# szuwgh/whisper.rs

Measured on AMD Instinct MI355X. Metric: real-time factor + encoder ms, Whisper-base 30s audio, 1 GPU and 8-GPU batch, higher is better.
Workload: dtype f16; 1 GPU; whisper-base f16 (random-init ggml-v1 weights), 1 x 30 s synthetic clip(s) per GPU: mel + conv stem + encoder + cross-KV + 128 greedy tokens; beam=0, clips_per_gpu=1, global_clips=1, n_decode=128, parallelism=1 GPU

## Files before the change

### whisper.rs_amd/csrc/wmi_api.cpp

```cpp
#include <hip/hip_runtime.h>
#include <rccl/rccl.h>

#include <math.h>
#include <stdarg.h>
#include <stdio.h>
#include <stdlib.h>
#include <string.h>

#include <algorithm>
#include <map>
#include <memory>
#include <set>
#include <string>
#include <vector>

#include "../../include/whisper_mi355x.h"
#include "wmi_host.h"
#include "wmi_internal.h"

#pragma clang fp contract(off)

using namespace wmi;

namespace {
// ... 113 lines not shown
    size_t tt_tsum_cap = 0;
    float *tt_pcm = nullptr;
    size_t tt_pcm_cap = 0;
    char *tt_spans = nullptr;
    size_t tt_spans_cap = 0;
    struct TokTime { int64_t t0, t1; float vlen; };
    struct Segment { int64_t t0, t1; int first, count; std::string text; };
    struct SegList {
        std::vector<Segment> segments;
        std::vector<TsRec> tokens;
        std::vector<TokTime> times;
    };
    std::vector<SegList> results = std::vector<SegList>(1);
    std::vector<int32_t> ts_prompt;
    int n_lang = 0;
    int task = WMI_TASK_TRANSCRIBE;
    std::vector<int32_t> lang_set;
    std::vector<int32_t> lang_used;
    std::vector<float> lang_p;
    bool lang_default = true, lang_any_auto = false;
    int32_t *d_lang = nullptr;
    int32_t *d_lang_auto = nullptr, *d_lang_det = nullptr;
    float *d_lang_p = nullptr, *d_lang_probs = nullptr;
    uint32_t *derr = nullptr;
    size_t sync_bytes = 0;
    int s_stride = 0, n_chunks_max = 0;
    unsigned long long *damax = nullptr;
    DecState *dstate = nullptr;
    int32_t *dfeed = nullptr;
    int feed_cap = 0;
    int32_t *dtokens = nullptr;
    size_t tokens_cap = 0;
    std::vector<float *> pcm_dev;
    std::vector<size_t> pcm_cap;
    float **d_pcm_ptrs = nullptr;
    int64_t *d_nsamp = nullptr, *d_nlen = nullptr;
    uint32_t *d_melmax = nullptr;
    float *d_mel = nullptr;
    size_t mel_cap = 0;
    int64_t mel_stride = 0, max_len = 0;
    std::vector<int64_t> n_len_host, n_samp_host;
    std::map<int32_t, float *> au_taps;
    void *au_raw = nullptr;
    float *au_mono = nullptr;
    size_t au_raw_cap = 0, au_mono_cap = 0;
    long long au_chunk = AUDIO_CHUNK_MAX;
    std::vector<hipEvent_t> au_ev;
    float au_ms = 0.0f;
    int au_converted = 0;
    int n_clips = 0;
    int enc_T = 0;
    int enc_clips = 0;
    int layout_T = -1;
    int cur_ctx = 0;
    int staged_n_decode = 0;
    std::vector<std::vector<int32_t>> staged_beam;
    hipEvent_t ev[8] = {};
    wmi_timings timings{};
    struct Graph { hipGraph_t graph = nullptr; hipGraphExec_t exec = nullptr; };
    std::map<std::string, Graph> graphs;
    void clear_graphs() {
        for (auto &kv : graphs) {
            if (kv.second.exec) (void)hipGraphExecDestroy(kv.second.exec);
            if (kv.second.graph) (void)hipGraphDestroy(kv.second.graph);
        }
        graphs.clear();
    }
    bool use_graph = true;
    bool use_coop = true;
    Tune tune;
    bool checksums = false;
    float cks[5] = {0, 0, 0, 0, 0};
    bool use_persist = true;
    int persist_q5 = -1;
    bool persist_logits = false;
    float *d_lgall = nullptr;
    int lg_rows = 0;
    int dec_layers = 0;
    int enc_layers = 0;
    int fault_inject = 0;
    bool persist_vreg = true;
    bool use_xshare = true;
    int early_ops = 1;
    int split_rows = 8;
    hipStream_t stream2 = nullptr;
    hipEvent_t ev_fork = nullptr, ev_join = nullptr;
    uint64_t *d_xg2 = nullptr;
    DecState *dstate2 = nullptr;
    int n_fallbacks = 0;
    PersistLayer *d_players = nullptr;
    uint32_t *d_expfb = nullptr;
    float gelu_min = __builtin_huge_valf();
    int n_expfb = 0;
    uint64_t *d_xg = nullptr;
    size_t xg_bytes = 0;
    int32_t *d_curtok = nullptr;
    int persist_G[9] = {-1, -1, -1, -1, -1, -1, -1, -1, -1};
    int persist_nres[9] = {};
    unsigned long long *d_ptrace = nullptr;
    ncclComm_t comm = nullptr;
    int rank = 0, world = 1;
    int32_t *d_gather = nullptr;
    int32_t *d_dsend = nullptr;
    int32_t *d_dctl = nullptr;
    int32_t *d_dbar = nullptr, *d_dshape = nullptr;
    size_t gather_cap = 0;
};

static float gelu_min_of(const wmi_context *ctx) { return ctx->tune.gelu_calc ? ctx->gelu_min : __builtin_huge_valf(); }

namespace {

int set_err(wmi_context *ctx, int code, const char *fmt, ...) {
    char buf[1024];
    va_list ap;
    va_start(ap, fmt);
    vsnprintf(buf, sizeof(buf), fmt, ap);
    va_end(ap);
    if (ctx) ctx->last_error = buf;
    g_last_error = buf;
    return code;
}

#define HIPCHK(ctx, expr)                                                                        \
    do {                                                                                         \
        hipError_t _e = (expr);                                                                  \
        if (_e != hipSuccess)                                                                    \
            return set_err((ctx), WMI_E_HIP, "HIP error %s at %s:%d: %s", hipGetErrorName(_e),    \
                           __FILE__, __LINE__, #expr);                                           \
    } while (0)

#define RCCLCHK(ctx, expr)                                                                       \
    do {                                                                                         \
        ncclResult_t _r = (expr);                                                                \
        if (_r != ncclSuccess)                                                                   \
            return set_err((ctx), WMI_E_RCCL, "RCCL error %s at %s:%d", ncclGetErrorString(_r),    \
                           __FILE__, __LINE__);                                                  \
    } while (0)

int prompt_tokens(const wmi_context *ctx, int32_t *out) {
    int n = 0;
    out[n++] = ctx->sp.sot;
    if (ctx->sp.is_multilingual) {
        out[n++] = ctx->sp.sot + 1;
        out[n++] = ctx->task == WMI_TASK_TRANSLATE ? ctx->sp.translate : ctx->sp.transcribe;
    }
    out[n++] = ctx->sp.not_;
    return n;
}

const char *const kLangCodes[LANG_MAX] = {
    "en", "zh", "de", "es", "ru", "ko", "fr", "ja", "pt", "tr", "pl", "ca", "nl", "ar", "sv", "it", "id", "hi", "fi", "vi",
    "he", "uk", "el", "ms", "cs", "ro", "da", "hu", "ta", "no", "th", "ur", "hr", "bg", "lt", "la", "mi", "ml", "cy", "sk",
    "te", "fa", "lv", "bn", "sr", "az", "sl", "kn", "et", "mk", "br", "eu", "is", "hy", "ne", "mn", "bs", "kk", "sq", "sw",
    "gl", "mr", "pa", "si", "km", "sn", "yo", "so", "af", "oc", "ka", "be", "tg", "sd", "gu", "am", "yi", "lo", "uz", "fo",
    "ht", "ps", "tk", "nn", "mt", "sa", "lb", "my", "bo", "tl", "mg", "as", "tt", "haw", "ln", "ha", "ba", "jw", "su", "yue",
};

struct Arena {
    size_t off = 0;
    std::vector<std::pair<size_t, size_t>> dummy;
    size_t take(size_t bytes) {
        const size_t o = off;
        off = up(off + bytes, 256);
        return o;
    }
// ... 1069 lines not shown
                    if (pd) pw[kk] += (double)((long long)pd - (long long)prev) * 0.01;
                    prev = v;
                }
            tot += (double)(prev - s0) * 0.01;
            ++ns;
        }
        if (!ns) return WMI_OK;
        double l1 = 0, l2 = 0, l3 = 0;
        for (int st = 1; st < steps; ++st) {
            const unsigned long long e = at(st, L - 1, 10, w);
            l1 += (double)(at(st, L, 1, w) - e) * 0.01;
            l2 += (double)(at(st, L, 2, w) - e) * 0.01;
            l3 += (double)(at(st, L, 3, w) - e) * 0.01;
        }
        fprintf(stderr, "[wmi ptrace] wg %s: logits LN done %.2f, resident rows done %.2f, streamed rows done %.2f us\n",
                wname[w], l1 / ns, l2 / ns, l3 / ns);
        if (steps > 2) {
            const double dc = (double)(at(steps - 1, L, 4, w) - at(1, L, 4, w));
            const double dt = (double)(at(steps - 1, L, 0, w) - at(1, L, 0, w)) * 10e-9;
            fprintf(stderr, "[wmi ptrace] wg %s: shader clock %.3f GHz\n", wname[w], dc / dt * 1e-9);
        }
        fprintf(stderr, "[wmi ptrace] wg %s: step %.2f us; per phase (per layer) total / until input arrived:\n", wname[w], tot / ns);
        for (int k = 0; k < 12; ++k) {
            const double d = k < 11 ? (double)ns * L : (double)ns;
            fprintf(stderr, "[wmi ptrace]   %-9s %6.2f / %6.2f\n", nm[k], ph[k] / d, pw[k] / d);
        }
        for (int k = 11; k < 32; ++k) {
            if (k == 16) k = 27;
            double s = 0;
            int c = 0;
            for (int st = 1; st < steps; ++st)
                for (int l = 0; l < L; ++l) {
                    const unsigned long long v = at(st, l, k, w);
                    unsigned long long pd = 0;
                    for (int j = 16; j < 27; ++j) {
                        const unsigned long long p = at(st, l, j, w);
                        if (p && p <= v && p > pd) pd = p;
                    }
                    if (v && pd) { s += (double)(v - pd) * 0.01; ++c; }
                }
            if (c) fprintf(stderr, "[wmi ptrace]   sub %d: %6.2f us after poll\n", k, s / c);
        }
    }
    return WMI_OK;
}

int persist_grid_for(wmi_context *ctx, int B) {
    if (!ctx->use_persist || B < 1 || B > 8) return 0;
    if (ctx->persist_G[B] < 0)
        ctx->persist_G[B] = persist_grid(ctx->device, ctx->hp.n_text_state, B, ctx->hp.n_audio_ctx, ctx->hp.n_vocab,
                                         &ctx->persist_nres[B]);
    return ctx->persist_G[B];
}

PersistArgs persist_args(wmi_context *ctx, const DecRun &run, int G) {
    const wmi_hparams &hp = ctx->hp;
    const int n = hp.n_text_state, H = hp.n_text_head, T = ctx->enc_T;
    const int b0 = run.b0, B = run.B, out_stride = run.out_stride;
    const bool beam = run.kind == RUN_BEAM;
    PersistArgs a{};
    a.layers = ctx->d_players; a.te = ctx->te; a.pe = ctx->d_pe; a.dln_w = ctx->dln_w; a.dln_b = ctx->dln_b;
    a.gelu_tab = ctx->gelu_tab; a.exp_tab = ctx->exp_tab; a.n_exp = ctx->n_exp; a.exp_fb = ctx->d_expfb;
    a.gelu_min = gelu_min_of(ctx);
    a.kcache = ctx->kcache; a.vcache = ctx->vcache; a.ck = ctx->ck; a.cv = ctx->cv;
    a.L = ctx->dec_layers; a.n = n; a.V = hp.n_vocab; a.B = B; a.T = T; a.tctx = hp.n_text_ctx;
    a.Bt = ctx->enc_clips; a.b0 = b0;
    const int rows_t = beam && n > 768 && ctx->use_xshare && (int64_t)H * ((T + 127) / 128) <= G ? 1 : B;
    const int cl_max = B == 1 && !beam ? 256 : 512;
    int cl = 128;
    while (cl < cl_max &&
           ((int64_t)rows_t * H * ((T + cl - 1) / cl) > G || (int64_t)B * H * ((T + cl - 1) / cl) > PX_TASKS))
        cl += 128;
    a.cl = cl;
    a.nch = (T + cl - 1) / cl;
    a.xshare = rows_t == 1 && B > 1 ? 1 : 0;
    a.qscale = powf((float)n / (float)H, -0.25f);
    a.st = ctx->dstate; a.feed = ctx->dfeed; a.feed_len = run.feed_len; a.feed_stride = run.feed_stride;
    a.tokens_out = ctx->dtokens + (size_t)b0 * out_stride; a.out_stride = out_stride;
    a.cur_tok = ctx->d_curtok; a.suppress_id = run.suppress_eot ? ctx->sp.eot : -1;
    a.xg = ctx->d_xg; a.err = ctx->derr;
    a.nres = ctx->persist_nres[B];
    a.vreg = ctx->persist_vreg ? 1 : 0;
    a.early_ops = ctx->early_ops;
    a.stall_wg = -1;
    if (ctx->fault_inject == 1) {
        a.stall_wg = G - 1;
        ctx->fault_inject = 2;
    }
    a.logits_out = ctx->d_lgall ? ctx->d_lgall + (size_t)b0 * hp.n_vocab : ctx->persist_logits ? ctx->dlogits : nullptr;
    a.lg_stride = ctx->d_lgall ? (int64_t)ctx->lg_rows * hp.n_vocab : 0;
    const bool have5 = ctx->use_q5 && !ctx->dec.empty() && ctx->dec[0].wqkv5;
    a.q5 = have5 && ctx->persist_q5 != 0 ? 1 : 0;
    if (run.kind == RUN_GREEDY) return a;
    a.n_steps = 1;
    a.logits_out = ctx->dlogits;
    a.lg_stride = 0;
    if (beam) {
        a.beam = 1;
        a.cur_tok = ctx->dbstate->tok;
        a.kv_src = ctx->dkvsrc;
        a.kv_src_stride = hp.n_text_ctx;
        a.tokens_out = ctx->dtokens;
    } else {
        a.out_stride = 0;
        if (run.kind == RUN_TS) a.cur_tok = ctx->dts_tok;
    }
    return a;
}

int reset_run(wmi_context *ctx, bool first, int G, int Gh, bool err_cleared, const int32_t *feed, int n_feed,
              bool ts = false, bool ruled = false) {
    ResetArgs ra{};
    auto zero = [&](void *p, size_t bytes) {
        ra.ptr[ra.n] = p;
        ra.bytes[ra.n++] = bytes;
    };
    if (feed && n_feed <= 64) {
        ra.dfeed = ctx->dfeed;
        ra.n_feed = n_feed;
        for (int i = 0; i < n_feed; ++i) ra.feed[i] = feed[i];
    } else if (feed) {
        HIPCHK(ctx, hipMemcpyAsync(ctx->dfeed, feed, (size_t)n_feed * 4, hipMemcpyHostToDevice, ctx->stream));
    }
    if (first && !err_cleared) zero(ctx->derr, 4);
    zero(ctx->dstate, sizeof(DecState));
    zero(ctx->damax, 8 * AMAX_SHARDS * 8);
    zero(ctx->dsync, ctx->sync_bytes);
    if (ts) zero(ctx->dts_done, DEC_ROWS * 4 + (ruled ? DEC_ROWS * sizeof(RuleHist) : 0));
    if (G > 0) zero(ctx->d_xg, ctx->xg_bytes);
    if (Gh > 0) {
        zero(ctx->d_xg2, ctx->xg_bytes);
        zero(ctx->dstate2, sizeof(DecState));
    }
    HIPCHK(ctx, launch_dec_reset(ctx->stream, ra));
    return WMI_OK;
}

struct RunGrid { int G, Gh; };
RunGrid run_grid(wmi_context *ctx, const DecRun &run) {
    const int G = persist_grid_for(ctx, run.B);
    const bool split = run.kind == RUN_GREEDY && G > 0 && ctx->split_rows > 1 && run.B >= ctx->split_rows;
    return {G, split ? persist_split_grid(ctx->hp.n_text_state, G) : 0};
}

int advance_run(wmi_context *ctx, const DecRun &run, RunGrid gr, int pos0, int steps) {
    const wmi_hparams &hp = ctx->hp;
    const int G = gr.G, Gh = gr.Gh;
    if (G <= 0) return run_dec_steps(ctx, run, pos0, steps);
    if (run.kind != RUN_GREEDY) {
        for (int i = 0; i < steps; ++i) {
            PersistArgs pa = persist_args(ctx, run, G);
            const int s_all = pos0 + i;
            if (run.kind == RUN_BEAM && ctx->d_ptrace && run.b0 == 0 && s_all < hp.n_text_ctx)
                pa.ptrace = ctx->d_ptrace + (size_t)s_all * (hp.n_text_layer + 1) * 32 * 2;
            HIPCHK(ctx, launch_dec_persist(ctx->stream, pa, G));
            if (run.kind == RUN_BEAM && ctx->d_lgall && s_all < hp.n_text_ctx)
                HIPCHK(ctx, hipMemcpyAsync(ctx->d_lgall + (size_t)s_all * ctx->lg_rows * hp.n_vocab, ctx->dlogits,
                                           (size_t)run.K * hp.n_vocab * 4, hipMemcpyDeviceToDevice, ctx->stream));
            if (run.kind == RUN_TS && run.sampled && ctx->d_lgall && s_all < hp.n_text_ctx && run.b0 + run.B <= ctx->lg_rows)
                HIPCHK(ctx, hipMemcpyAsync(ctx->d_lgall + ((size_t)s_all * ctx->lg_rows + run.b0) * hp.n_vocab, ctx->dlogits,
                                           (size_t)run.B * hp.n_vocab * 4, hipMemcpyDeviceToDevice, ctx->stream));
            int rc = enqueue_step_tail(ctx, run);
            if (rc) return rc;
        }
        return WMI_OK;
    }
// ... 993 lines not shown
        out->clear();
        if (t > 0) *out = beam_backtrack(hpar, hrec, t - 1, bs.fin_beam[pk.i]);
        out->push_back(frec[pk.i]);
        if (score) *score = bs.fin_score[pk.i];
    } else {
        *out = beam_backtrack(hpar, hrec, ns - 1, pk.i);
        if (score) *score = bs.score[pk.i];
    }
    return WMI_OK;
}

}

template <typename F>
int guarded(wmi_context *ctx, F &&f) {
    try {
        return f();
    } catch (const std::bad_alloc &) {
        return set_err(ctx, WMI_E_UNEXPECTED, "host memory exhausted");
    } catch (const std::exception &e) {
        return set_err(ctx, WMI_E_UNEXPECTED, "internal error: %s", e.what());
    } catch (...) {
        return set_err(ctx, WMI_E_UNEXPECTED, "internal error");
    }
}

extern "C" {

const char *wmi_last_error(const wmi_context *ctx) { return ctx ? ctx->last_error.c_str() : g_last_error.c_str(); }
const char *wmi_last_error_global(void) { return g_last_error.c_str(); }

static int wmi_init_from_file_impl(const char *path, int device, int max_clips, wmi_context **out) {
    if (!out || !path) return set_err(nullptr, WMI_E_INVALID_ARG, "null argument");
    *out = nullptr;
    if (max_clips < 1) return set_err(nullptr, WMI_E_INVALID_ARG, "max_clips must be >= 1");
    ParsedModel pm;
    std::string err;
    int rc = parse_file(path, pm, err);
    if (rc) return set_err(nullptr, rc, "%s", err.c_str());
    int ndev = 0;
    if (hipGetDeviceCount(&ndev) != hipSuccess || ndev <= 0)
        return set_err(nullptr, WMI_E_HIP, "no HIP device available (the MI355X path has no CPU fallback)");
    if (device < 0 || device >= ndev) return set_err(nullptr, WMI_E_INVALID_ARG, "device %d of %d", device, ndev);
    std::unique_ptr<wmi_context> ctx(new wmi_context());
    ctx->device = device;
    ctx->max_clips = max_clips;
    ctx->hp = pm.hp;
    ctx->wf32 = pm.hp.f16 % 1000 == 0;
    init_specials(pm.hp.n_vocab, ctx->sp);
    ctx->n_lang = ctx->sp.is_multilingual ? std::min(LANG_MAX, std::max(0, ctx->sp.translate - (ctx->sp.sot + 1))) : 0;
    ctx->lang_set.assign(max_clips, 0);
    ctx->lang_used.assign(max_clips, 0);
    ctx->lang_p.assign(max_clips, -1.0f);
    ctx->vocab = std::move(pm.vocab);
    for (int32_t i = (int32_t)ctx->vocab.size(); i < pm.hp.n_vocab; ++i) {
        char b[64];
        if (i > ctx->sp.beg) snprintf(b, sizeof b, "[_TT_%d]", i - ctx->sp.beg);
        else if (i == ctx->sp.eot) snprintf(b, sizeof b, "[_EOT_]");
        else if (i == ctx->sp.sot) snprintf(b, sizeof b, "[_SOT_]");
        else if (i == ctx->sp.prev) snprintf(b, sizeof b, "[_PREV_]");
        else if (i == ctx->sp.not_) snprintf(b, sizeof b, "[_NOT_]");
        else if (i == ctx->sp.beg) snprintf(b, sizeof b, "[_BEG_]");
        else snprintf(b, sizeof b, "[_extra_token_%d]", i);
        ctx->vocab.push_back(b);
    }
    HIPCHK(ctx.get(), hipSetDevice(device));
    HIPCHK(ctx.get(), hipStreamCreateWithFlags(&ctx->stream, hipStreamNonBlocking));
    rc = upload_model(ctx.get(), pm);
    if (rc) { g_last_error = ctx->last_error; wmi_free(ctx.release()); return rc; }
    pm.tensors.clear();
    rc = alloc_workspace(ctx.get());
    if (rc) { g_last_error = ctx->last_error; wmi_free(ctx.release()); return rc; }
    if (getenv("WMI_NO_GRAPH")) ctx->use_graph = false;
    if (getenv("WMI_NO_COOP")) ctx->use_coop = false;
    if (getenv("WMI_NO_Q5")) ctx->use_q5 = false;
    if (getenv("WMI_NO_FUSE")) ctx->fuse_wo = false;
    if (const char *c = getenv("WMI_PERSIST")) ctx->use_persist = ctx->use_persist && atoi(c) != 0;
    if (getenv("WMI_PERSIST_LOGITS")) ctx->persist_logits = true;
    if (const char *e = getenv("WMI_PERSIST_Q5")) ctx->persist_q5 = atoi(e) ? 1 : 0;
    if (const char *c = getenv("WMI_CHECKSUMS")) ctx->checksums = atoi(c) != 0;
    if (const char *c = getenv("WMI_FAULT_INJECT")) ctx->fault_inject = atoi(c) ? 1 : 0;
    if (const char *c = getenv("WMI_XSHARE")) ctx->use_xshare = atoi(c) != 0;
    if (const char *c = getenv("WMI_EARLY_OPERANDS")) ctx->early_ops = atoi(c) != 0;
    if (const char *c = getenv("WMI_SPLIT_ROWS")) ctx->split_rows = atoi(c);
    if (const char *c = getenv("WMI_AUDIO_CHUNK")) ctx->au_chunk = std::max(1ll, std::min(atoll(c), AUDIO_CHUNK_MAX));
    ctx->dec_layers = ctx->hp.n_text_layer;
    if (const char *c = getenv("WMI_DEC_LAYERS")) ctx->dec_layers = std::max(1, std::min(atoi(c), ctx->hp.n_text_layer));
    ctx->enc_layers = ctx->hp.n_audio_layer;
    if (const char *c = getenv("WMI_ENC_LAYERS")) ctx->enc_layers = std::max(0, std::min(atoi(c), ctx->hp.n_audio_layer));
    if (const char *c = getenv("WMI_LOGITS_ALL"); c && atoi(c)) {
        ctx->lg_rows = std::max(DEC_ROWS, max_clips);
        const size_t nb = (size_t)ctx->hp.n_text_ctx * ctx->lg_rows * ctx->hp.n_vocab * 4;
        HIPCHK(ctx.get(), hipMalloc(&ctx->d_lgall, nb));
        HIPCHK(ctx.get(), hipMemset(ctx->d_lgall, 0, nb));
    }
    if (getenv("WMI_PTRACE")) {
        const size_t nb = (size_t)hp_ptrace_slots(ctx->hp) * 8;
        HIPCHK(ctx.get(), hipMalloc(&ctx->d_ptrace, nb));
        HIPCHK(ctx.get(), hipMemset(ctx->d_ptrace, 0, nb));
    }
    Tune &tn = ctx->tune;
    auto knob = [](const char *name, int &v, int lo) {
        if (const char *c = getenv(name)) {
            const int x = atoi(c);
            if (x >= lo) v = x;
        }
    };
    knob("WMI_LOGITS_CAP", tn.logits_cap, 1);
    knob("WMI_GRAPH_STEPS", tn.graph_steps, 1);
    knob("WMI_XATTN_ROWS", tn.xattn_rows, 0);
    knob("WMI_ENC_ATTN_NW", tn.enc_attn_nw, 0);
    knob("WMI_GEMM_G", tn.gemm_g, 0);
    knob("WMI_GEMM_EPI", tn.epi_staged, 0);
    knob("WMI_GEMM_P", tn.gemm_p, 0);
    knob("WMI_GELU_CALC", tn.gelu_calc, 0);
    knob("WMI_MEL_G", tn.mel_g, 0);
    knob("WMI_GEMM32_TILE", tn.gemm32_tile, 0);
    *out = ctx.release();
    return WMI_OK;
}

void wmi_free(wmi_context *ctx) {
    if (!ctx) return;
    (void)hipSetDevice(ctx->device);
    if (ctx->stream) (void)hipStreamSynchronize(ctx->stream);
    if (ctx->comm) (void)ncclCommDestroy(ctx->comm);
    ctx->clear_graphs();
    for (float *p : ctx->pcm_dev) if (p) (void)hipFree(p);
    for (auto &kv : ctx->au_taps) if (kv.second) (void)hipFree(kv.second);
    if (ctx->au_raw) (void)hipFree(ctx->au_raw);
    if (ctx->au_mono) (void)hipFree(ctx->au_mono);
    for (hipEvent_t e : ctx->au_ev) (void)hipEventDestroy(e);
    for (uint32_t *p : ctx->tt_E) if (p) (void)hipFree(p);
    for (unsigned long long *p : ctx->tt_P) if (p) (void)hipFree(p);
    if (ctx->tt_tsum) (void)hipFree(ctx->tt_tsum);
    if (ctx->tt_pcm) (void)hipFree(ctx->tt_pcm);
    if (ctx->tt_spans) (void)hipFree(ctx->tt_spans);
    if (ctx->d_mel) (void)hipFree(ctx->d_mel);
    if (ctx->dfeed) (void)hipFree(ctx->dfeed);
    if (ctx->dtokens) (void)hipFree(ctx->dtokens);
    if (ctx->d_gather) (void)hipFree(ctx->d_gather);
    if (ctx->d_dsend) (void)hipFree(ctx->d_dsend);
    if (ctx->d_dctl) (void)hipFree(ctx->d_dctl);
    if (ctx->d_ws) (void)hipFree(ctx->d_ws);
    if (ctx->d_model) (void)hipFree(ctx->d_model);
    if (ctx->d_players) (void)hipFree(ctx->d_players);
    if (ctx->d_expfb) (void)hipFree(ctx->d_expfb);
    if (ctx->d_ptrace) (void)hipFree(ctx->d_ptrace);
    if (ctx->d_lgall) (void)hipFree(ctx->d_lgall);
    if (ctx->d_lang) (void)hipFree(ctx->d_lang);
    if (ctx->dts_tok) (void)hipFree(ctx->dts_tok);
    if (ctx->dts_rec) (void)hipFree(ctx->dts_rec);
    if (ctx->d_tsb_parts) (void)hipFree(ctx->d_tsb_parts);
    if (ctx->d_tsb_rec) (void)hipFree(ctx->d_tsb_rec);
    if (ctx->d_win) (void)hipFree(ctx->d_win);
    if (ctx->d_samp_rows) (void)hipFree(ctx->d_samp_rows);
    if (ctx->d_rule_m0) (void)hipFree(ctx->d_rule_m0);
    for (auto &e : ctx->ev) if (e) (void)hipEventDestroy(e);
    if (ctx->stream) (void)hipStreamDestroy(ctx->stream);
    if (ctx->stream2) (void)hipStreamDestroy(ctx->stream2);
    if (ctx->ev_fork) (void)hipEventDestroy(ctx->ev_fork);
    if (ctx->ev_join) (void)hipEventDestroy(ctx->ev_join);
    delete ctx;
}

int wmi_get_hparams(const wmi_context *ctx, wmi_hparams *out) {
// ... 1220 lines not shown
```

### whisper.rs_amd/csrc/wmi_internal.h

```cpp
#pragma once
#include <hip/hip_runtime.h>
#include <stdint.h>

namespace wmi {

hipError_t launch_selftest(hipStream_t s, const uint16_t *exp_tab, int n_exp, uint32_t *mismatch);

struct MelTables {
    float hann[400];
    float c400[200], s400[200], c200[100], s200[100], c100[50], s100[50], c50[25], s50[25];
    float dc[625], ds[625];
};
static_assert(sizeof(MelTables) % 16 == 0, "k_mel_frames copies MelTables in 16-byte chunks");

hipError_t launch_mel_frames(hipStream_t s, const MelTables *tabs, const float *filt_t , int n_mel,
                             const float *const *pcm, const int64_t *n_samples, float *mel, int64_t mel_stride,
                             const int64_t *n_len, int64_t max_len, uint32_t *mel_max, int n_clips,
                             const float *filt_c , int n_fc);
constexpr int MEL_FC_MAX = 4096;
struct ResetArgs {
    void *ptr[8];
    size_t bytes[8];
    int n;
    int32_t *dfeed;
// ... 314 lines not shown
    int out_stride;
    const DecState *st;
    int n, B, record_only;
};
hipError_t launch_dec_embed(hipStream_t s, const DecEmbedArgs &a);

struct PersistLayer {
    const float *ln1_w, *ln1_b;
    const uint16_t *wqkv; const float *bqkv;
    const uint16_t *wo; const float *bo;
    const float *lnc_w, *lnc_b;
    const uint16_t *wcq; const float *bcq;
    const uint16_t *wco; const float *bco;
    const float *ln2_w, *ln2_b;
    const uint16_t *w0; const float *b0;
    const uint16_t *w1; const float *b1;
    const uint8_t *wqkv5, *wo5, *wco5, *w05, *w15;
};

struct XLayout {
    int x1, x2, x3, q, k, v, o, xq, oc, h, s, p, a, ctl, total;
};
constexpr int PX_TASKS = 2048;
constexpr int PX_GMAX = 256;
__host__ __device__ inline XLayout persist_layout(int n, int H, int T) {
    XLayout L{};
    int o = 0;
    const int R = 8;
    L.x1 = o; o += R * n;
    L.x2 = o; o += R * n;
    L.x3 = o; o += R * n;
    L.q = o; o += R * n / 2;
    L.k = o; o += R * n / 2;
    L.v = o; o += R * n / 2;
    L.o = o; o += R * n / 2;
    L.xq = o; o += R * n / 2;
    L.oc = o; o += R * n / 2;
    L.h = o; o += R * 2 * n;
    L.s = o; o += 3 * R * H * ((T + 127) / 128);
    L.p = o; o += R * H * ((T + 127) / 128) * 64;
    L.a = o; o += R * PX_GMAX * 2;
    L.ctl = o; o += 16;
    L.total = (o + 15) / 16 * 16;
    return L;
}

struct PersistArgs {
    const PersistLayer *layers;
    const uint16_t *te;
    const float *pe;
    const float *dln_w, *dln_b;
    const uint16_t *gelu_tab;
    float gelu_min = __builtin_huge_valf();
    const uint16_t *exp_tab;
    int n_exp;
    const uint32_t *exp_fb;
    uint16_t *kcache, *vcache;
    const uint16_t *ck, *cv;
    int L, n, V, B, T, tctx, Bt, b0;
    int nch, cl;
    float qscale;
    DecState *st;
    const int32_t *feed;
    int feed_len, feed_stride;
    int32_t *tokens_out;
    int out_stride;
    int32_t *cur_tok;
    int suppress_id;
    int n_steps;
    uint64_t *xg;
    uint32_t *err;
    unsigned long long *ptrace;
    int nres;
    float *logits_out;
    int64_t lg_stride;
    int beam;
    const int32_t *kv_src;
    int kv_src_stride;
    int q5;
    int xshare;
    int stall_wg;
    int vreg;
    int early_ops;
};
__host__ __device__ constexpr bool px_e_early(bool early, int H, int ntask, int G) { return early && H + ntask <= G; }
__host__ __device__ constexpr int px_e_first_task(bool early, int wg, int H, int ntask, int G) {
    return px_e_early(early, H, ntask, G) ? (wg >= H ? wg - H : ntask) : wg;
}
constexpr bool px_e_tasks_once(bool early, int H, int nch, int G) {
    const int ntask = H * nch;
    for (int t = 0; t < ntask; ++t) {
        int cnt = 0;
        for (int wg = 0; wg < G; ++wg)
            for (int u = px_e_first_task(early, wg, H, ntask, G); u < ntask; u += G) cnt += u == t;
        if (cnt != 1) return false;
    }
    return true;
}
static_assert(px_e_tasks_once(true, 2, 12, 256) && px_e_tasks_once(true, 6, 12, 256) && px_e_tasks_once(true, 8, 12, 256) &&
                  px_e_tasks_once(true, 12, 12, 256) && px_e_tasks_once(true, 12, 12, 192) && px_e_tasks_once(true, 2, 1, 256),
              "cross tasks beside the self-attention workgroups");
static_assert(px_e_tasks_once(true, 12, 24, 192) && px_e_tasks_once(false, 8, 12, 256) && px_e_tasks_once(false, 12, 12, 64),
              "cross tasks where they do not fit beside them, or the knob is off");
constexpr int PX_EOP_NMAX = 512;
inline int persist_trace_wg(const PersistArgs &a, int G) {
    const int H = a.n / 64;
    return a.B == 1 && !a.beam && a.n <= PX_EOP_NMAX && px_e_early(a.early_ops != 0, H, H * a.nch, G) ? H : G / 2;
}
hipError_t launch_dec_persist(hipStream_t s, const PersistArgs &a, int G);
hipError_t launch_exp_fallbacks(hipStream_t s, const uint16_t *exp_tab, int n_exp, uint32_t *list, uint32_t *n);
hipError_t launch_persist_selftest(hipStream_t s, const uint16_t *exp_tab, int n_exp, const uint32_t *fb,
                                   uint32_t *mismatch);
int persist_grid(int device, int n, int B, int T, int V, int *nres);
int persist_split_grid(int n, int G);

}
```

### whisper.rs_amd/csrc/wmi_persist.hip

```cpp
#include <hip/hip_runtime.h>

#include <type_traits>

#include "wmi_device.h"
#include "wmi_internal.h"

#pragma clang fp contract(off)

namespace wmi {
hipError_t launch_persist_q5(hipStream_t s, const PersistArgs &a, int G);
int grid_persist_q5(int device, int n, int B, int V, int *nres);

namespace {

constexpr int PT = 256;
constexpr uint32_t PSPIN = 1u << 19;
constexpr int NPH = 11;
constexpr int PMAXB = 8;
constexpr int RNMAX = 16;
__host__ __device__ constexpr int scr_bytes(int BT) { return BT == 1 ? 8 * 1024 : 24 * 1024; }
constexpr int NKP = 4;
constexpr int EXPFB = 64;
constexpr int XS_OFF = 1024;
constexpr int XS_BYTES = 8192;
// ... 216 lines not shown
    if constexpr (NP > 1 && BT * KCH <= 32) {
        float acc[NP][BT];
#pragma unroll
        for (int p = 0; p < NP; ++p)
#pragma unroll
            for (int b = 0; b < BT; ++b) acc[p][b] = 0.0f;
        if constexpr (BT == 1 && KCH <= 8 && KCH >= PRE_GEMV_MIN) {
            half8 xa[KCH];
            xs_chunks(xa, xs, 0, l16);
#pragma unroll
            for (int c = 0; c < KCH; ++c)
#pragma unroll
                for (int p = 0; p < NP; ++p) acc[p][0] = dot8(wc_h8(S.w[p][c], sh), xa[c], acc[p][0]);
        } else
#pragma unroll
        for (int c = 0; c < KCH; ++c) {
            half8 xv[BT];
#pragma unroll
            for (int b = 0; b < BT; ++b)
                if (b < B) xv[b] = *(const half8 *)(xs + b * K + c * 128 + l16 * 8);
#pragma unroll
            for (int p = 0; p < NP; ++p) {
                const half8 wv = wc_h8(S.w[p][c], sh);
#pragma unroll
                for (int b = 0; b < BT; ++b)
                    if (b < B) acc[p][b] = dot8(wv, xv[b], acc[p][b]);
            }
        }
#pragma unroll
        for (int p = 0; p < NP; ++p) {
            float v = 0.0f;
#pragma unroll
            for (int b = 0; b < BT; ++b)
                if (b < B) {
                    const float t = red16_sum(acc[p][b]);
                    if (l16 == b) v = t;
                }
            acc[p][0] = v;
        }
#pragma unroll
        for (int p = 0; p < NP; ++p) {
            if (rb + 16 * p >= r1) break;
            const int row = rb + 16 * p + slot;
            epi(row, l16, acc[p][0], S.bias[p], row < r1 && l16 < B);
        }
        return;
    }
#pragma unroll
    for (int p = 0; p < NP; ++p) {
        if (rb + 16 * p >= r1) break;
        const int row = rb + 16 * p + slot;
        float acc[BT];
#pragma unroll
        for (int b = 0; b < BT; ++b) acc[b] = 0.0f;
#pragma unroll
        for (int c = 0; c < KCH; ++c) {
            const half8 wv = wc_h8(S.w[p][c], sh);
#pragma unroll
            for (int b = 0; b < BT; ++b)
                if (b < B) acc[b] = dot8(wv, *(const half8 *)(xs + b * K + c * 128 + l16 * 8), acc[b]);
        }
        float v = 0.0f;
#pragma unroll
        for (int b = 0; b < BT; ++b)
            if (b < B) {
                float t = acc[b];
                t = red16_sum(t);
                if (l16 == b) v = t;
            }
        epi(row, l16, v, S.bias[p], row < r1 && l16 < B);
    }
}

template <int KCH, int KS, bool Q5 = false>
struct WSplit {
    static constexpr int CQ = (KCH + KS - 1) / KS;
    WChunk<Q5> w[CQ];
};
#ifndef WMI_GDESIGN
#define WMI_GDESIGN PX_GMAX
#endif
constexpr int PX_GDESIGN = WMI_GDESIGN;
static_assert(PX_GDESIGN >= 32 && PX_GDESIGN <= PX_GMAX, "design grid");
__host__ __device__ constexpr int rows_full(int N) { return (((N + PX_GDESIGN - 1) / PX_GDESIGN) + 1) & ~1; }
__host__ __device__ constexpr int split_of(int kch, int rows) {
    int best = 1;
    for (int k = 1; k <= kch; ++k)
        if (kch % k == 0 && rows * k <= 16) best = k;
    return best;
}

template <int KCH, int KS, bool Q5>
__device__ __forceinline__ void wsplit_pre(WSplit<KCH, KS, Q5> &S, int l16) {
#pragma unroll
    for (int c = 0; c < WSplit<KCH, KS, Q5>::CQ; ++c) wc_pre(S.w[c], (l16 & 3) * 8);
}

template <int KCH, int KS, bool Q5>
__device__ __forceinline__ void wsplit_load(WSplit<KCH, KS, Q5> &S, const WMat &m, int K, int rb, int r1, int slot,
                                            int l16) {
    constexpr int CQ = WSplit<KCH, KS, Q5>::CQ;
    const int rl = slot / KS, ks = slot - rl * KS, row = rb + rl;
    const bool ok = rl < 16 / KS && row < r1;
    const int64_t e0 = (int64_t)(ok ? row : 0) * K + ks * CQ * 128 + l16 * 8;
#pragma unroll
    for (int c = 0; c < CQ; ++c) wc_zero(S.w[c]);
    if (ok) {
#pragma unroll
        for (int c = 0; c < CQ; ++c) wc_load(S.w[c], m, e0 + c * 128);
    }
}

template <int KS, bool PAIR>
constexpr bool wsplit_inwave() { return KS == 2 || (KS == 4 && !PAIR); }
template <int KS>
__device__ __forceinline__ int wsplit_row(int w, int q) {
    if constexpr (KS == 2) return q < 2 ? 2 * w + q : -1;
    else return q == 0 ? w : -1;
}

template <int BT, int KCH, int KS, bool Q5, bool PAIR = true, typename Epi>
__device__ __forceinline__ void wsplit_dot(const WSplit<KCH, KS, Q5> &S, const f16 *xs, int K, int B, int rb, int r1,
                                           int slot, int l16, float bias, float *kpart, Epi &&epi) {
    constexpr int CQ = WSplit<KCH, KS, Q5>::CQ;
    const int rl = slot / KS, ks = slot - rl * KS, sh = (l16 & 3) * 8;
    float acc[BT];
#pragma unroll
    for (int b = 0; b < BT; ++b) acc[b] = 0.0f;
    if constexpr (BT == 1 && CQ <= 8 && CQ >= PRE_GEMV_MIN) {
        half8 xa[CQ];
        xs_chunks(xa, xs, ks * CQ, l16);
#pragma unroll
        for (int c = 0; c < CQ; ++c) acc[0] = dot8(wc_h8(S.w[c], sh), xa[c], acc[0]);
    } else
#pragma unroll
    for (int c = 0; c < CQ; ++c) {
        const half8 wv = wc_h8(S.w[c], sh);
#pragma unroll
        for (int b = 0; b < BT; ++b)
            if (b < B) acc[b] = dot8(wv, *(const half8 *)(xs + b * K + (ks * CQ + c) * 128 + l16 * 8), acc[b]);
    }
    float v = 0.0f;
#pragma unroll
    for (int b = 0; b < BT; ++b)
        if (b < B) {
            const float t = red16_sum(acc[b]);
            if (l16 == b) v = t;
        }
    if constexpr (wsplit_inwave<KS, PAIR>()) {
        const int w = slot >> 2, q = slot & 3;
        uint32_t a0, a1, c0, c1;
        swap16(__float_as_uint(v), a0, a1);
        float sum;
        if constexpr (KS == 2) {
            sum = v + __uint_as_float(a1);
            swap32(__float_as_uint(sum), c0, c1);
            swap16(c1, a0, a1);
            sum = q == 1 ? __uint_as_float(a0) : sum;
        } else {
            uint32_t d0, d1;
            swap32(__float_as_uint(v), c0, c1);
            swap32(a1, d0, d1);
            sum = ((v + __uint_as_float(a1)) + __uint_as_float(c1)) + __uint_as_float(d1);
        }
        const int rloc = wsplit_row<KS>(w, q);
        const int row = rb + (rloc < 0 ? 0 : rloc);
        epi(row, l16, sum, bias, rloc >= 0 && row < r1 && l16 < B);
        return;
    }
    if (l16 < PMAXB && rl < 16 / KS) kpart[(rl * KS + ks) * PMAXB + l16] = v;
    __syncthreads();
    const int row = rb + slot;
    float sum = 0.0f;
// ... 324 lines not shown
    const uint16_t hr = f2h_bits(r);
    hv = h2f_bits(hr);
    const float nb = h2f_bits(r >= hv ? (uint16_t)(hr + 1) : (uint16_t)(hr - 1));
    const float mid = 0.5f * (hv + nb);
    const float ulp = __uint_as_float(__float_as_uint(r) & 0x7f800000u) * 1.1920928955078125e-7f;
    return fabsf(r - mid) > 4.0f * ulp;
}
__device__ __forceinline__ float exp_f16_hash(float arg, const uint32_t *fbt, uint32_t K) {
    const f16 hx = (f16)arg;
    const float hv = h2f_bits(f2h_bits(expf((float)hx)));
    const uint32_t j = __builtin_bit_cast(uint16_t, hx) & 0x7fff;
    const uint32_t e = fbt[(j * K) >> 26];
    return (e >> 16) == j ? h2f_bits((uint16_t)e) : hv;
}

#define PHASE_IDS                                                                              \
    int tid = (int)threadIdx.x;                                                                \
    asm volatile("" : "+v"(tid) : : "memory");                                                 \
    const int lane = tid & 63, w = tid >> 6, q = lane >> 4, l16 = lane & 15, slot = w * 4 + q; \
    (void)q; (void)l16; (void)slot;

#define PTWG (EOP && eop ? H : G / 2)
#define PSTAMP(ph)                                                                                    \
    if (a.ptrace && threadIdx.x == 0 && (wg == 0 || wg == PTWG))                                      \
        a.ptrace[(((int64_t)step * (L + 1) + (ph) / 32) * 32 + ((ph) & 31)) * 2 + (wg == 0 ? 0 : 1)] = \
            __builtin_amdgcn_s_memrealtime();

#define PREFETCH_ISSUED asm volatile("" : : : "memory");

template <int NS, int NKE, bool ON>
struct XOps {
    half8 kf[NKE][4], vf[NKE][4];
    WSet<NS / 128, 4> S;
    Ln1P<NS> l1;
};
template <int NS, int NKE>
struct XOps<NS, NKE, false> {};

template <int NS, int BT, bool BEAM, bool Q5>
__global__ __launch_bounds__(PT, 1) void k_dec_persist(PersistArgs a) {
    constexpr int KC = NS / 128;
    constexpr int H = NS / 64;
    constexpr int NPL = KC <= 4 ? 2 : 1;
    constexpr bool LMF = KC <= 4;
    constexpr bool LMF2 = !LMF && BT > 1;
    constexpr bool XQF = KC <= 6;
    constexpr int NKE = BT == 1 ? 2 : NKP;
    const bool xsh = BEAM && !XQF && a.xshare;
    constexpr int KS_N = split_of(KC, rows_full(NS)), KS_I = split_of(4 * KC, rows_full(NS));
    constexpr int KS_A = split_of(KC, rows_full(3 * NS)), KS_H = split_of(KC, rows_full(4 * NS));
    extern __shared__ __attribute__((aligned(16))) unsigned char smem[];
    __shared__ PShared sh;
    const int B = BT == 1 ? 1 : a.B, G = gridDim.x, wg = blockIdx.x;
    if (wg == a.stall_wg) return;
    const int tid = threadIdx.x, lane = tid & 63, w = tid >> 6;
    const int L = a.L, T = a.T, tctx = a.tctx, nch = a.nch, CL = a.cl;
    const int nsub = (T + 127) >> 7;
    constexpr bool EOP = BT == 1 && XQF && NS <= PX_EOP_NMAX;
    const bool eop = EOP && px_e_early(a.early_ops != 0, H, H * nch, G);
    const int et0 = EOP ? px_e_first_task(eop, wg, H, H * nch, G) : wg;
    constexpr int PUX = BT == 1 ? (NS <= 1024 ? 4 : 8) : 16;
    constexpr int PUH = BT == 1 ? (NS <= 512 ? 4 : NS <= 1024 ? 8 : 16) : 16;
    float *xf = (float *)smem;
    f16 *xs = (f16 *)(smem + (size_t)B * NS * 4);
    unsigned char *scr = smem + (size_t)B * NS * 4 + (size_t)B * NS * 8;
    f16 *vres = (f16 *)(scr + scr_bytes(BT));
    int oX1, oX2, oX3, oQ, oK, oV, oO, oXQ, oOC, oH, oS, oP, oA;
    {
        const XLayout X = persist_layout(NS, H, T);
        oX1 = X.x1; oX2 = X.x2; oX3 = X.x3; oQ = X.q; oK = X.k; oV = X.v; oO = X.o; oXQ = X.xq;
        oOC = X.oc; oH = X.h; oS = X.s; oP = X.p; oA = X.a;
    }
    uint64_t *xg = a.xg;
    uint32_t *abortw = (uint32_t *)(xg + persist_layout(NS, H, T).ctl);
    const float qs = a.qscale;
    auto part = [&](int N, bool even, int &r0, int &r1) {
        int rpw = (N + G - 1) / G;
        if (even) rpw = (rpw + 1) & ~1;
        r0 = wg * rpw < N ? wg * rpw : N;
        r1 = r0 + rpw < N ? r0 + rpw : N;
    };
    int rn0, rn1, ra0, ra1, rh0, rh1, rv0, rv1;
    part(NS, true, rn0, rn1);
    part(3 * NS, true, ra0, ra1);
    part(4 * NS, true, rh0, rh1);
    float *kpbuf = BT > 1 ? (float *)scr : sh.kpart;
    part(a.V, false, rv0, rv1);
    const int rn = rn1 - rn0;
    const int rs0 = rv0 + a.nres < rv1 ? rv0 + a.nres : rv1;
    {
        const uint4 *src = (const uint4 *)((const f16 *)a.te + (int64_t)rv0 * NS);
        uint4 *dst = (uint4 *)vres;
        for (int i = tid; i < (rs0 - rv0) * NS / 8; i += PT) {
            const int j = i / (NS / 8), c = i - j * (NS / 8);
            dst[LMF || LMF2 ? j * (NS / 8) + (c ^ (j & 15)) : i] = src[i];
        }
    }
    constexpr bool LREG2 = BT == 1 && !LMF && !LMF2 && KC <= 6;
    const bool lreg2 = LREG2 && a.vreg && rv1 - rs0 <= 128;
    WSet<LREG2 ? KC : 1, LREG2 ? 8 : 1> SR;
    if constexpr (LREG2) wset_load(SR, wmat(a.te), nullptr, NS, rs0, lreg2 ? rv1 : rs0, w * 4 + (lane >> 4), lane & 15);
    if (tid == 0) sh.abort_ = 0;
    if (tid < EXPFB) sh.expfb[tid] = a.exp_fb[tid];
    const uint32_t fbk = a.exp_fb[EXPFB + 1];
    __syncthreads();
    auto check = [&](bool ok) -> bool {
        if (!ok) sh.abort_ = 1;
        __syncthreads();
        return sh.abort_ != 0;
    };
    auto ptr_u64 = [](uint64_t *base) { return [base](int i) { return base + i; }; };

    auto argmax_gather = [&](int pp) -> bool {
        uint32_t *ga = (uint32_t *)scr;
        const bool ok = gpoll<BT == 1 ? 4 : 16>(B * G * 2, atag(pp, L), ptr_u64(xg + oA), ga, abortw, a.err);
        if (check(ok)) return false;
        for (int b = 0; b < B; ++b) {
            unsigned long long k = 0ull;
            if (tid < G) k = ((unsigned long long)ga[(b * G + tid) * 2] << 32) | ga[(b * G + tid) * 2 + 1];
            k = wave_max_u64(k);
            if (lane == 0) sh.best[w][b] = k;
        }
        __syncthreads();
        if (tid < B) {
            unsigned long long k = sh.best[0][tid];
            for (int i = 1; i < 4; ++i) k = sh.best[i][tid] > k ? sh.best[i][tid] : k;
            sh.tok[tid] = (int32_t)(0xffffffffu - (uint32_t)(k & 0xffffffffull));
        }
        __syncthreads();
        return true;
    };

    auto xk_load = [&](int l, int t, int tid, half8 (&kf)[NKE][4]) {
        const int c = t % nch, bh = t / nch, h = bh % H, b = bh / H;
        const int j0 = c * CL, j1 = j0 + CL < T ? j0 + CL : T;
        const int64_t cb = ((int64_t)l * a.Bt + a.b0 + (a.beam ? 0 : b)) * T * NS + h * 64;
        const f16 *Kb = (const f16 *)a.ck + cb + (tid & 1) * 32;
        const half8 z8 = {};
#pragma unroll
        for (int p = 0; p < NKE; ++p) {
            int key = j0 + 128 * p + (tid >> 1);
            key = key < j1 ? key : j1 - 1;
#pragma unroll
            for (int i = 0; i < 4; ++i)
                kf[p][i] = 128 * p < CL ? sld((const half8 *)(Kb + (int64_t)key * NS + 8 * i)) : z8;
        }
    };
    auto xv_load = [&](int l, int t, int tid, half8 (&vf)[NKE][4]) {
        const int c = t % nch, bh = t / nch, h = bh % H, b = bh / H;
        const int j0 = c * CL, j1 = j0 + CL < T ? j0 + CL : T;
        const int64_t cb = ((int64_t)l * a.Bt + a.b0 + (a.beam ? 0 : b)) * T * NS + h * 64;
        const int doct = tid & 7, jg = tid >> 3;
        const f16 *Vb = (const f16 *)a.cv + cb + doct * 8;
        const half8 z8 = {};
#pragma unroll
        for (int p = 0; p < NKE; ++p)
#pragma unroll
            for (int u = 0; u < 4; ++u) {
                int kv = j0 + 128 * p + jg * 4 + u;
                kv = kv < j1 ? kv : j1 - 1;
                vf[p][u] = 128 * p < CL ? sld((const half8 *)(Vb + (int64_t)kv * NS)) : z8;
            }
    };

    int pos = a.st->pos;
    for (int step = 0; step < a.n_steps; ++step, ++pos) {
        for (int l = 0; l < L; ++l) {
            ConstLayer &P = ((ConstLayer *)a.layers)[l];
            uint16_t *kc = a.kcache + (size_t)l * DEC_ROWS * tctx * NS;
            uint16_t *vc = a.vcache + (size_t)l * DEC_ROWS * tctx * NS;

            {
                PHASE_IDS
                const uint32_t tag = ptag(pos, L, l, 0);
                PSet<NS, BT, KC, 2, KS_A, Q5> S;
                const bool act = ra0 < ra1;
                const bool late_w = !Q5 && l == 0 && pos >= a.feed_len && step > 0;
                if (!late_w) S.load(lmat<Q5>(P.wqkv, P.wqkv5, 3 * NS * NS), P.bqkv, NS, ra0, ra1, slot, l16);
                LnP<NS> lp;
                Ln1P<NS> l1;
                if constexpr (BT == 1) ln1_params<NS>(P.ln1_w, P.ln1_b, l1, tid);
                else ln_params_early<NS>(P.ln1_w, P.ln1_b, lp, lane);
                PREFETCH_ISSUED
                __syncthreads();
                if (l == 0) {
                    const bool fed = pos < a.feed_len;
                    if (fed) {
                        if (tid < B) sh.tok[tid] = a.feed[tid * a.feed_stride + pos];
                        __syncthreads();
                    } else if (step == 0) {
                        if (tid < B) sh.tok[tid] = a.cur_tok[tid];
                        __syncthreads();
                    } else {
                        if (!argmax_gather(pos - 1)) return;
                        S.load(lmat<Q5>(P.wqkv, P.wqkv5, 3 * NS * NS), P.bqkv, NS, ra0, ra1, slot, l16);
                        if (wg == 0 && tid < B && pos - a.feed_len < a.out_stride)
                            a.tokens_out[tid * a.out_stride + (pos - a.feed_len)] = sh.tok[tid];
                    }
                    S.pre(l16);
                    for (int i = tid; i < B * NS / 4; i += PT) {
                        const int b = (i * 4) / NS, e = i * 4 - b * NS;
                        const half4 tv = *(const half4 *)((const f16 *)a.te + (int64_t)sh.tok[b] * NS + e);
                        const float4 pv = *(const float4 *)(a.pe + (int64_t)pos * NS + e);
                        *(float4 *)(xf + b * NS + e) = make_float4((float)tv[0] + pv.x, (float)tv[1] + pv.y,
                                                                   (float)tv[2] + pv.z, (float)tv[3] + pv.w);
                    }
                    if constexpr (BT == 1) {
                        __syncthreads();
                        float xv[Ln1P<NS>::NE];
#pragma unroll
                        for (int u = 0; u < Ln1P<NS>::NE; ++u) xv[u] = xf[tid + PT * u < NS ? tid + PT * u : 0];
                        if (!ln1_vals<NS>(xv, l1, xs, true, sh.redd, sh.redd2, &sh.abort_)) return;
                    }
                } else {
                    if constexpr (BT == 1) {
                        if (!poll_ln1<NS>(xg + oX1, ptag(pos, L, l - 1, 10), l1, xf, xs, abortw, a.err, sh.redd, sh.redd2,
                                          &sh.abort_, [&] { S.pre(l16); }))
                            return;
                    } else {
                        const bool ok = gpoll<PUX>(B * NS, ptag(pos, L, l - 1, 10), ptr_u64(xg + oX1), (uint32_t *)xf, abortw, a.err,
                                                   [&] { S.pre(l16); });
                        if (check(ok)) return;
                    }
                PSTAMP(l * 32 + 16)
                }
                __syncthreads();
                for (int i = tid; i < B * rn; i += PT) {
                    const int b = i / rn, r = i - b * rn;
                    sh.xres[b][r] = xf[b * NS + rn0 + r];
                }
                if constexpr (BT > 1) {
                    ln_rows<NS>(xf, lp, xs, B, w, lane);
                    __syncthreads();
                }
                PSTAMP(l * 32 + 27)
                if (act)
                    S.template dot<BT>(xs, NS, B, ra0, ra1, slot, l16, kpbuf, [&](int row, int b, float v, float eb, bool valid) {
                        const float vn = from_next_row(v), ebn = from_next_row(eb);
                        if (!valid || (q & 1)) return;
                        const int which = row / NS, c = row - which * NS;
                        uint32_t pk;
                        if (which == 0) pk = pack2((v + eb) * qs, (vn + ebn) * qs);
                        else if (which == 1) pk = pack2(v * qs, vn * qs);
                        else pk = pack2(eb + v, ebn + vn);
                        const int64_t gi = (which == 0 ? oQ : which == 1 ? oK : oV) + b * (NS / 2) + c / 2;
                        if (which > 0)
                            st32((uint32_t *)((which == 1 ? kc : vc) + ((int64_t)b * tctx + pos) * NS + c), pk);
                        gput(xg + gi, tag, pk);
                    });
            }

            PSTAMP(l * 32 + 0)
            {
                PHASE_IDS
// ... 1099 lines not shown
```

Measured before the change: 1988 audio-s/s (x real-time; 1/RTF).

## Place Wqkv projection rows off the self-attention workgroups in persistent decoder

In the persistent decoder kernel with batch 1 and no beam search, the fused QKV projection rows are now assigned only to workgroups beyond the first H, the ones that run self-attention heads. Those head workgroups skip the QKV phase and only do the token and embedding setup for layer 0. This is meant to let the attention workgroups start earlier and to shorten the critical path. In exchange, each remaining workgroup takes slightly more rows. Compile-time checks confirm the new row partition covers every row exactly once, and an environment knob can turn it off.

```diff
diff --git a/whisper.rs_amd/csrc/wmi_api.cpp b/whisper.rs_amd/csrc/wmi_api.cpp
--- a/whisper.rs_amd/csrc/wmi_api.cpp
+++ b/whisper.rs_amd/csrc/wmi_api.cpp
@@ -219,6 +219,7 @@
     bool persist_vreg = true;
     bool use_xshare = true;
     int early_ops = 1;
+    int a_off_b = 1;
     int split_rows = 8;
     hipStream_t stream2 = nullptr;
     hipEvent_t ev_fork = nullptr, ev_join = nullptr;
@@ -1454,6 +1455,7 @@
     a.nres = ctx->persist_nres[B];
     a.vreg = ctx->persist_vreg ? 1 : 0;
     a.early_ops = ctx->early_ops;
+    a.a_off_b = ctx->a_off_b;
     a.stall_wg = -1;
     if (ctx->fault_inject == 1) {
         a.stall_wg = G - 1;
@@ -2613,6 +2615,7 @@
     if (const char *c = getenv("WMI_FAULT_INJECT")) ctx->fault_inject = atoi(c) ? 1 : 0;
     if (const char *c = getenv("WMI_XSHARE")) ctx->use_xshare = atoi(c) != 0;
     if (const char *c = getenv("WMI_EARLY_OPERANDS")) ctx->early_ops = atoi(c) != 0;
+    if (const char *c = getenv("WMI_A_OFF_B")) ctx->a_off_b = atoi(c) != 0;
     if (const char *c = getenv("WMI_SPLIT_ROWS")) ctx->split_rows = atoi(c);
     if (const char *c = getenv("WMI_AUDIO_CHUNK")) ctx->au_chunk = std::max(1ll, std::min(atoll(c), AUDIO_CHUNK_MAX));
     ctx->dec_layers = ctx->hp.n_text_layer;
diff --git a/whisper.rs_amd/csrc/wmi_internal.h b/whisper.rs_amd/csrc/wmi_internal.h
--- a/whisper.rs_amd/csrc/wmi_internal.h
+++ b/whisper.rs_amd/csrc/wmi_internal.h
@@ -420,7 +420,51 @@
     int stall_wg;
     int vreg;
     int early_ops;
-};
+    int a_off_b;
+};
+__host__ __device__ constexpr int px_rows_even(int N, int G) { return (((N + G - 1) / G) + 1) & ~1; }
+__host__ __device__ constexpr int split_of(int kch, int rows) {
+    int best = 1;
+    for (int k = 1; k <= kch; ++k)
+        if (kch % k == 0 && rows * k <= 16) best = k;
+    return best;
+}
+__host__ __device__ constexpr bool px_a_off_b(bool on, int n, int H, int G, int GD) {
+    if (!on || G <= H) return false;
+    const int N = 3 * n, old = px_rows_even(N, G), rpw = px_rows_even(N, G - H);
+    const int ks = split_of(n / 128, px_rows_even(N, GD));
+    return ks > 1 ? rpw * ks <= 16 : split_of(n / 128, rpw) == 1 && (rpw + 15) / 16 <= (old + 15) / 16;
+}
+__host__ __device__ constexpr int px_a_rpw(bool off_b, int n, int H, int G) {
+    return px_rows_even(3 * n, off_b ? G - H : G);
+}
+__host__ __device__ constexpr int px_a_row0(bool off_b, int wg, int n, int H, int G) {
+    const int s = off_b ? wg - H : wg, r = s * px_a_rpw(off_b, n, H, G);
+    return s >= 0 && r < 3 * n ? r : 3 * n;
+}
+constexpr bool px_a_rows_once(bool want, int n, int G, int GD) {
+    const int H = n / 64, N = 3 * n;
+    const bool ob = px_a_off_b(true, n, H, G, GD);
+    if (ob != want) return false;
+    int next = 0;
+    for (int wg = 0; wg < G; ++wg) {
+        const int r0 = px_a_row0(ob, wg, n, H, G), r1 = r0 + px_a_rpw(ob, n, H, G) < N ? r0 + px_a_rpw(ob, n, H, G) : N;
+        if (r0 == N) continue;
+        if ((ob && wg < H) || r0 != next || (r0 & 1) || r1 <= r0) return false;
+        next = r1;
+    }
+    return next == N;
+}
+static_assert(px_a_rows_once(true, 128, 256, 256) && px_a_rows_once(true, 384, 256, 256) && px_a_rows_once(true, 512, 256, 256) &&
+                  px_a_rows_once(true, 768, 256, 256) && px_a_rows_once(true, 1024, 256, 256),
+              "Wqkv rows off the self-attention workgroups");
+static_assert(px_a_rpw(true, 128, 2, 256) == 2 && px_a_rpw(true, 384, 6, 256) == 6 && px_a_rpw(true, 512, 8, 256) == 8 &&
+                  px_a_rpw(true, 768, 12, 256) == 10 && px_a_rpw(true, 1024, 16, 256) == 14,
+              "rows per workgroup of the placement");
+static_assert(px_a_rows_once(false, 1280, 256, 256) && px_a_rows_once(false, 512, 192, 192) && px_a_rows_once(false, 512, 64, 256) &&
+                  !px_a_off_b(false, 512, 8, 256, 256),
+              "the partition over all workgroups where the rows would not fit, or the knob is off");
+constexpr int PX_AOB_NMAX = 1024;
 __host__ __device__ constexpr bool px_e_early(bool early, int H, int ntask, int G) { return early && H + ntask <= G; }
 __host__ __device__ constexpr int px_e_first_task(bool early, int wg, int H, int ntask, int G) {
     return px_e_early(early, H, ntask, G) ? (wg >= H ? wg - H : ntask) : wg;
diff --git a/whisper.rs_amd/csrc/wmi_persist.hip b/whisper.rs_amd/csrc/wmi_persist.hip
--- a/whisper.rs_amd/csrc/wmi_persist.hip
+++ b/whisper.rs_amd/csrc/wmi_persist.hip
@@ -322,13 +322,7 @@
 #endif
 constexpr int PX_GDESIGN = WMI_GDESIGN;
 static_assert(PX_GDESIGN >= 32 && PX_GDESIGN <= PX_GMAX, "design grid");
-__host__ __device__ constexpr int rows_full(int N) { return (((N + PX_GDESIGN - 1) / PX_GDESIGN) + 1) & ~1; }
-__host__ __device__ constexpr int split_of(int kch, int rows) {
-    int best = 1;
-    for (int k = 1; k <= kch; ++k)
-        if (kch % k == 0 && rows * k <= 16) best = k;
-    return best;
-}
+__host__ __device__ constexpr int rows_full(int N) { return px_rows_even(N, PX_GDESIGN); }
 
 template <int KCH, int KS, bool Q5>
 __device__ __forceinline__ void wsplit_pre(WSplit<KCH, KS, Q5> &S, int l16) {
@@ -819,7 +813,14 @@
     };
     int rn0, rn1, ra0, ra1, rh0, rh1, rv0, rv1;
     part(NS, true, rn0, rn1);
-    part(3 * NS, true, ra0, ra1);
+    constexpr bool AOB = BT == 1 && !BEAM && NS <= PX_AOB_NMAX;
+    const bool aob = AOB && px_a_off_b(a.a_off_b != 0, NS, H, G, PX_GDESIGN);
+    if constexpr (AOB) {
+        ra0 = px_a_row0(aob, wg, NS, H, G);
+        ra1 = ra0 + px_a_rpw(aob, NS, H, G) < 3 * NS ? ra0 + px_a_rpw(aob, NS, H, G) : 3 * NS;
+    } else {
+        part(3 * NS, true, ra0, ra1);
+    }
     part(4 * NS, true, rh0, rh1);
     float *kpbuf = BT > 1 ? (float *)scr : sh.kpart;
     part(a.V, false, rv0, rv1);
@@ -907,6 +908,26 @@
             uint16_t *kc = a.kcache + (size_t)l * DEC_ROWS * tctx * NS;
             uint16_t *vc = a.vcache + (size_t)l * DEC_ROWS * tctx * NS;
 
+            if (AOB && aob && ra0 >= ra1) {
+                if (l == 0) {
+                    PHASE_IDS
+                    __syncthreads();
+                    if (pos < a.feed_len) {
+                        if (tid < B) sh.tok[tid] = a.feed[tid * a.feed_stride + pos];
+                        __syncthreads();
+                    } else if (step == 0) {
+                        if (tid < B) sh.tok[tid] = a.cur_tok[tid];
+                        __syncthreads();
+                    } else {
+                        if (!argmax_gather(pos - 1)) return;
+                        if (wg == 0 && tid < B && pos - a.feed_len < a.out_stride)
+                            a.tokens_out[tid * a.out_stride + (pos - a.feed_len)] = sh.tok[tid];
+                    }
+                    for (int r = tid; r < rn; r += PT)
+                        sh.xres[0][r] = (float)((const f16 *)a.te)[(int64_t)sh.tok[0] * NS + rn0 + r] +
+                                        a.pe[(int64_t)pos * NS + rn0 + r];
+                }
+            } else
             {
                 PHASE_IDS
                 const uint32_t tag = ptag(pos, L, l, 0);
```

New measurement: 2053 audio-s/s (x real-time; 1/RTF), median of 6. +3.3%, better.
